# hbdat/cvpr22_cross_modal_pseudo_labeling

Measured on AMD Instinct MI355X. Metric: images/sec student-teacher train step (COCO 800x1333), higher is better.
Workload: dtype f32 (bf16x3 split MFMA, fp32 accum); 1 GPU; student_teacher_mask_rcnn_uncertainty.yaml R-50-C4, 2 img/GPU 3x800x1333, fwd+bwd+allreduce+SGD; global_batch=2, parallelism=dp1, losses_finite=True, pipelined=True

## Files before the change

### cvpr22_cross_modal_pseudo_labeling_amd/_C.py

```python
import contextlib
import functools
import ctypes
import threading

import torch

from . import _cpu, _lib

_L = _lib.load()


def _stream():
    return torch._C._cuda_getCurrentRawStream(torch.cuda.current_device())


class _Same:

    def __enter__(self):
        return None

    def __exit__(self, *exc):
        return False


# ... 789 lines not shown
        raise RuntimeError("split_gemm_pair: residual must be a float32 [M, N] HIP tensor with unit column stride")
    with _on(dev):
        config = _gemm_cfg(config)
        nbytes = _gemm_ws_bytes(m, n, ch, ch2, kh, kw, w, config) if not (config & 8) else 0
        ws = torch.empty((nbytes,), dtype=torch.uint8, device=dev) if nbytes else None
        rc = _L.ovis_split_gemm_pair(a_pair.data_ptr(), 2 * a_pair.stride(0),
                                     0 if a2_pair is None else a2_pair.data_ptr(),
                                     0 if a2_pair is None else 2 * a2_pair.stride(0),
                                     b_pair.data_ptr(), 2 * b_pair.stride(0),
                                     0 if c is None else c.data_ptr(), n, 0 if cp is None else cp.data_ptr(), 4 * n,
                                     0 if bias is None else bias.data_ptr(),
                                     0 if residual is None else residual.data_ptr(),
                                     0 if residual is None else residual.stride(0), m, n, ch, ch2, kh, kw, h, w,
                                     int(bool(flip)), int(bool(relu)), 0 if ws is None else ws.data_ptr(), nbytes,
                                     config, _stream())
    _lib.check(rc, "split_gemm_pair")
    return c, cp


def split_gemm_pair_pool_supported(m, n, ch, pool_rows):
    return bool(_L.ovis_split_gemm_pair_pool_supported(int(m), int(n), int(ch), int(pool_rows)))


def split_gemm_pair_rp_pool(a_pair, b_pair, bias, residual_pair, relu, out_f32, out_pair, pool_rows):
    for t, name in ((a_pair, "a_pair"), (b_pair, "b_pair")) + (((residual_pair, "residual_pair"),) if residual_pair is not None else ()):
        if not (t.is_cuda and t.dtype == torch.bfloat16 and t.dim() == 2 and t.stride(1) == 1):
            raise RuntimeError(f"split_gemm_pair_rp_pool: {name} must be a 2-D bfloat16 HIP tensor in pair layout")
    m, ch = a_pair.shape[0], a_pair.shape[1] // 2
    n, k = b_pair.shape[0], b_pair.shape[1] // 2
    if k != ch or m % pool_rows or (residual_pair is not None and residual_pair.shape != (m, 2 * n)):
        raise RuntimeError("split_gemm_pair_rp_pool: shape mismatch")
    dev = a_pair.device
    c = torch.empty((m, n), dtype=torch.float32, device=dev) if out_f32 else None
    cp = torch.empty((m, 2 * n), dtype=torch.bfloat16, device=dev) if out_pair else None
    pooled = torch.zeros((m // pool_rows, n), dtype=torch.float32, device=dev)
    if m == 0 or n == 0:
        return c, cp, pooled
    if bias is not None:
        bias = _dev(bias, "bias")
    with _on(dev):
        rc = _L.ovis_split_gemm_pair_rp_pool(a_pair.data_ptr(), 2 * a_pair.stride(0), b_pair.data_ptr(), 2 * b_pair.stride(0),
                                             0 if c is None else c.data_ptr(), n, 0 if cp is None else cp.data_ptr(), 4 * n,
                                             0 if bias is None else bias.data_ptr(),
                                             0 if residual_pair is None else residual_pair.data_ptr(),
                                             0 if residual_pair is None else 2 * residual_pair.stride(0), m, n, ch,
                                             int(bool(relu)), pooled.data_ptr(), int(pool_rows), 1.0 / pool_rows, _stream())
    _lib.check(rc, "split_gemm_pair_rp_pool")
    return c, cp, pooled


def weight_prep_pair(w, scale=None, want_transposed=False):
    if not (w.is_cuda and w.dtype == torch.float32 and w.dim() == 4):
        raise RuntimeError("weight_prep_pair: [N,C,KH,KW] float32 HIP tensor expected")
    w = w.detach().contiguous()
    n, c, kh, kw = w.shape
    t = kh * kw
    fwd = torch.empty((n, 2 * t * c), dtype=torch.bfloat16, device=w.device)
    bwd = torch.empty((c, 2 * t * n), dtype=torch.bfloat16, device=w.device) if want_transposed else None
    if scale is not None:
        scale = _dev(scale.detach(), "scale")
    with _on(w.device):
        rc = _L.ovis_weight_prep_pair_f32(w.data_ptr(), 0 if scale is None else scale.data_ptr(), fwd.data_ptr(),
                                          0 if bwd is None else bwd.data_ptr(), n, c, t, _stream())
    _lib.check(rc, "weight_prep_pair")
    return fwd, bwd


def split_gemm_pair_gated(a_pair, b_pair, gate_pair, conv=None, out_f32=False, out_pair=True, config=0):
    for t, name in ((a_pair, "a_pair"), (b_pair, "b_pair"), (gate_pair, "gate_pair")):
# ... 507 lines not shown
```

### cvpr22_cross_modal_pseudo_labeling_amd/_lib.py

```python
import ctypes
import os

_HERE = os.path.dirname(os.path.abspath(__file__))
LIB_PATH = os.path.join(_HERE, "libovis_hip.so")

OVIS_OK = 0
_ERRORS = {-1: "OVIS_EINVAL (bad size or null pointer)",
           -2: "OVIS_ENOSPC (workspace too small)",
           -3: "OVIS_ERANGE (problem size not supported by the kernel)"}

_vp, _i, _f, _sz, _l = ctypes.c_void_p, ctypes.c_int, ctypes.c_float, ctypes.c_size_t, ctypes.c_long

SIGNATURES = {
    "ovis_version": (ctypes.c_char_p, []),
    "ovis_roi_align_forward_f32": (_i, [_vp, _vp, _vp, _i, _i, _i, _i, _i, _i, _i, _f, _i, _vp]),
    "ovis_roi_align_forward_workspace_bytes": (_sz, [_i, _i, _i]),
    "ovis_roi_align_forward_mfma_supported": (_i, [_i, _i, _i, _i]),
    "ovis_roi_align_forward_ws_f32": (_i, [_vp, _vp, _vp, _i, _i, _i, _i, _i, _i, _i, _f, _i, _vp, _sz, _vp]),
    "ovis_roi_align_forward_strided_from_nhwc_f32": (_i, [_vp, _vp, _vp, _i, _i, _i, _i, _i, _i, _i, _i, _f, _i, _i, _vp]),
    "ovis_roi_align_backward_f32": (_i, [_vp, _vp, _vp, _i, _i, _i, _i, _i, _i, _i, _f, _i, _vp]),
    "ovis_roi_align_backward_workspace_bytes": (_sz, [_i, _i, _i, _i]),
    "ovis_roi_align_backward_plane_supported": (_i, [_i, _i, _i, _i]),
    "ovis_roi_align_backward_ws_f32": (_i, [_vp, _vp, _vp, _i, _i, _i, _i, _i, _i, _i, _f, _i, _vp, _sz, _vp]),
    "ovis_roi_align_backward_strided_ws_f32": (_i, [_vp, _vp, _vp, _i, _i, _i, _i, _i, _i, _i, _i, _f, _i, _vp, _sz, _vp]),
# ... 19 lines not shown
    "ovis_topk_sorted_f32": (_i, [_vp, _l, _i, _i, _i, _vp, _vp, _vp, _sz, _vp]),
    "ovis_rpn_decode_f32": (_i, [_vp, _l, _l, _l, _vp, _vp, _vp, _i, _i, _i, _i, _f, _f, _f, _f, _f, _f, _f, _vp, _vp, _vp]),
    "ovis_sigmoid_focal_loss_forward_f32": (_i, [_vp, _vp, _vp, _i, _i, _f, _f, _vp]),
    "ovis_sigmoid_focal_loss_backward_f32": (_i, [_vp, _vp, _vp, _vp, _i, _i, _f, _f, _vp]),
    "ovis_split_bf16x3_f32": (_i, [_vp, _l, _vp, _l, _i, _i, _vp]),
    "ovis_im2col_split_bf16x3_f32": (_i, [_vp, _vp, _l, _i, _i, _i, _i, _i, _i, _vp]),
    "ovis_bias_act_f32": (_i, [_vp, _vp, _vp, _l, _i, _i, _vp]),
    "ovis_split_pair_f32": (_i, [_vp, _l, _vp, _l, _i, _vp]),
    "ovis_gate_split_pair_rows_f32": (_i, [_vp, _l, _vp, _i, _vp, _vp, _l, _i, _vp, _i, _vp, _vp, _vp]),
    "ovis_gate_split_pair_f32": (_i, [_vp, _l, _vp, _i, _vp, _vp, _l, _i, _vp, _i, _vp]),
    "ovis_im2col_nchw_pair_f32": (_i, [_vp, _vp] + [_i] * 9 + [_vp]),
    "ovis_weight_prep_pair_f32": (_i, [_vp, _vp, _vp, _vp, _i, _i, _i, _vp]),
    "ovis_slab_reduce_f32": (_i, [_vp, _vp, _vp, _i, _i, _i, _i, _vp]),
    "ovis_im2col_pair": (_i, [_vp, _vp, _l, _i, _i, _i, _i, _i, _vp]),
    "ovis_split_gemm_tn_slices": (_i, [_l, _i, _i, _i]),
    "ovis_split_gemm_pair_tn": (_i, [_vp, _l, _vp, _l, _vp, _i, _l, _i, _i, _i, _i, _i, _i, _vp]),
    "ovis_split_gemm_pair_gated": (_i, [_vp, _l, _vp, _l, _vp, _l, _vp, _l, _vp, _l, _l] + [_i] * 8 + [_vp]),
    "ovis_split_gemm_pair_gated_ws": (_i, [_vp, _l, _vp, _l, _vp, _l, _vp, _l, _vp, _l, _l] + [_i] * 7 + [_vp, _sz, _i, _vp]),
    "ovis_split_gemm_pair_workspace_bytes": (_sz, [_l, _i, _i, _i, _i, _i, _i]),
    "ovis_split_gemm_pair_workspace_bytes_ex": (_sz, [_l, _i, _i, _i, _i, _i, _i, _i]),
    "ovis_split_gemm_pair_rp_gated": (_i, [_vp, _l, _vp, _l, _vp, _l, _vp, _l, _vp, _l, _vp, _l, _l, _i, _i, _i, _vp]),
    "ovis_split_gemm_pair_pool_supported": (_i, [_l, _i, _i, _i]),
    "ovis_split_gemm_pair_rp_pool": (_i, [_vp, _l, _vp, _l, _vp, _l, _vp, _l, _vp, _vp, _l, _l, _i, _i, _i, _vp, _i, _f, _vp]),
    "ovis_split_gemm_pair_rp": (_i, [_vp, _l, _vp, _l, _vp, _l, _vp, _l, _vp, _vp, _l, _l, _i, _i, _i, _vp, _sz, _i, _vp]),
    "ovis_split_gemm_pair": (_i, [_vp, _l, _vp, _l, _vp, _l, _vp, _l, _vp, _l, _vp, _vp, _l, _l] + [_i] * 9
                             + [_vp, _sz, _i, _vp]),
    "ovis_match_encode_f32": (_i, [_vp, _vp, _vp, _i, _i, _f, _f, _i, _f, _f, _f, _f, _vp, _vp, _vp, _vp]),
    "ovis_rpn_match_encode_f32": (_i, [_vp, _vp, _vp, _i, _i, _f, _f, _i, _f, _f, _f, _f, _vp, _vp, _vp, _vp]),
    "ovis_project_masks_f32": (_i, [_vp, _vp, _vp, _i, _i, _i, _i, _i, _vp, _vp]),
    "ovis_gemm_f32": (_i, [_vp, _l, _l, _vp, _l, _l, _vp, _vp, _l, _i, _i, _i, _vp]),
    "ovis_gemm_ex_f32": (_i, [_vp, _l, _l, _vp, _l, _l, _vp, _i, _f, _i, _vp, _l, _i, _i, _i, _vp]),
    "ovis_gemm_f32_workspace_bytes": (_sz, [_i, _i, _i]),
    "ovis_gemm_ex_ws_f32": (_i, [_vp, _l, _l, _vp, _l, _l, _vp, _i, _f, _i, _vp, _l, _i, _i, _i, _vp, _sz, _vp]),
    "ovis_deform_im2col_f32": (_i, [_vp, _vp, _vp, _vp] + [_i] * 13 + [_vp]),
    "ovis_deform_col2im_f32": (_i, [_vp, _vp, _vp, _vp] + [_i] * 13 + [_vp]),
    "ovis_deform_col2im_coord_f32": (_i, [_vp, _vp, _vp, _vp, _vp, _vp] + [_i] * 13 + [_vp]),
    "ovis_deform_im2col_pair_rows_f32": (_i, [_vp, _vp, _vp, _vp, _l] + [_i] * 15 + [_vp]),
    "ovis_deform_col2im_rows_f32": (_i, [_vp, _l, _vp, _vp, _vp, _vp, _vp, _vp] + [_i] * 15 + [_vp]),
    "ovis_region_noun_align_f32": (_i, [_vp, _vp, _vp, _vp, _vp, _i, _i, _i, _vp]),
    "ovis_text_embed_f32": (_i, [_vp, _l, _i, _vp, _vp, _i, _i, _vp, _vp]),
    "ovis_project_polygon_masks_f32": (_i, [_vp, _vp, _vp, _vp, _vp, _i, _i, _i, _i, _vp, _vp]),
    "ovis_sgd_momentum_multi_f32": (_i, [_vp, _vp, _i, _f, _f, _f, _i, _vp]),
    "ovis_bottleneck_identity_backward_workspace_bytes": (_sz, [_l, _i, _i, _i, _i, _i, _i]),
    "ovis_bottleneck_identity_backward": (_i, [_vp, _l] * 7 + [_vp] * 3 + [_l, _i, _i, _i, _i, _i, _i] + [_vp] * 7 + [_sz, _i, _vp, _vp]),
    "ovis_weight_prep_pair_multi_f32": (_i, [_vp, _vp, _i, _i, _vp]),
    "ovis_weight_prep_tile": (_i, []),
# ... 32 lines not shown
```

### cvpr22_cross_modal_pseudo_labeling_amd/csrc/split_gemm.hip

```cpp
#include <stdlib.h>

#include "ovis_common.h"
constexpr int kGroupWidth = 4;

namespace {
typedef short bf16x8 __attribute__((ext_vector_type(8)));
typedef float f32x4 __attribute__((ext_vector_type(4)));
typedef __bf16 b2 __attribute__((ext_vector_type(2)));
typedef float f2 __attribute__((ext_vector_type(2)));

__device__ char g_zero_line[128];

enum { PLAIN = 0, SHIFTED = 1, HALO = 2, DEFORM = 3 };
constexpr int kHalo = 8;

struct SplitGemmArgs {
  const char* A; long a_rs;
  const char* A2; long a2_rs;
  const char* B; long b_rs;
  float* C; long ldc;
  char* Cp; long cp_rs;
  const float* bias; const float* res; long ldr;
  const char* resp; long resp_rs;
  const char* gate; long gate_rs;
// ... 67 lines not shown
  }
  if (p.C) *(f32x4*)(p.C + m * p.ldc + n) = v;
  if (p.Cp) {
    const unsigned h01 = pack_bf16(v.x, v.y), h23 = pack_bf16(v.z, v.w);
    const unsigned l01 = pack_bf16(v.x - __uint_as_float(h01 << 16), v.y - __uint_as_float(h01 & 0xffff0000u));
    const unsigned l23 = pack_bf16(v.z - __uint_as_float(h23 << 16), v.w - __uint_as_float(h23 & 0xffff0000u));
    char* d = p.Cp + m * p.cp_rs + poff;
    *(uint2*)d = make_uint2(h01, h23);
    *(uint2*)(d + 64) = make_uint2(l01, l23);
  }
  return v;
}

__device__ __forceinline__ void epilogue_store4(const SplitGemmArgs& p, long m, int n, f32x4 v) {
  const long poff = (long)(n >> 5) * 128 + (n & 31) * 2;
  f32x4 bias4 = {0.f, 0.f, 0.f, 0.f};
  if (p.bias) bias4 = *(const f32x4*)(p.bias + n);
  const EpilogueSource src = epilogue_source(p);
  EpilogueOperands o;
  if (src.base) epilogue_fetch4(src, m, epilogue_column_bytes(p, n, poff), o);
  epilogue_apply4(p, m, n, poff, v, bias4, o);
}

template <int WM, int WN, int MODE, int NS, int OCC, bool DUAL = false, bool POOL = false>
__global__ __launch_bounds__(WM * WN * 64, OCC) void split_gemm_kernel(SplitGemmArgs p, int tiles_n, int ntiles) {
  constexpr int BM = WM * 64, BN = WN * 64, NW = WM * WN;
  constexpr int A_ROWS = MODE == HALO ? BM + 2 * kHalo + 2 : BM;
  constexpr int ZROW = BM + 2 * kHalo;
  constexpr int A_BYTES = A_ROWS * 128, B_BYTES = BN * 128, STAGE = A_BYTES + B_BYTES;
  constexpr int A_PIECES = (MODE == HALO ? BM + 2 * kHalo : BM) / 8;
  constexpr int AI = (A_PIECES + NW - 1) / NW;
  constexpr int BI = BN / 8 / NW;
  static_assert(MODE != HALO || NS == 1, "the halo tile is single-staged");
  static_assert(NW * 4096 <= STAGE * NS, "epilogue staging fits the k-loop's LDS");
  extern __shared__ __attribute__((aligned(16))) char smem[];

  const int lane = threadIdx.x & 63, wave = __builtin_amdgcn_readfirstlane(threadIdx.x >> 6);
  int id;
  {
    const int nblocks = gridDim.x;
    const int b = blockIdx.x, q = nblocks >> 3, r = nblocks & 7, xcd = b & 7, loc = b >> 3;
    id = (xcd < r ? xcd * (q + 1) : r * (q + 1) + (xcd - r) * q) + loc;
  }
  const int slice = id / ntiles;
  const int tile = id - slice * ntiles;
  const int gw = p.gw, tiles_m = ntiles / tiles_n;
  const int per_group = tiles_m * gw;
  const int grp = tile / per_group;
  const int in_grp = tile - grp * per_group;
  const int tile_m = in_grp / gw, tile_n = grp * gw + (in_grp - tile_m * gw);
  const long m0 = (long)tile_m * BM;
  const int n0 = tile_n * BN;
  const int Mi = (int)p.M;

  const int cpb = p.ch >> 5;
  const int nk = p.T * cpb + (p.ch2 >> 5);
  int dy = 0, dx = 0;
  auto set_tap = [&](int t) {
    dy = t / p.KW - p.KH / 2;
    dx = t % p.KW - p.KW / 2;
    if (p.flip) { dy = -dy; dx = -dx; }
  };

  struct LaneGeom { int lr, s0, s1; };
  auto lane_geom = [&](int ln) {
    const int lr = ln >> 3, lc = ln & 7;
// ... 328 lines not shown
              ps2 += rr >= pool_b2 ? fin : z;
            }
          }
        }
      }
    }
  }
  if constexpr (POOL) {
    f32x4* ps[3] = {&ps0, &ps1, &ps2};
#pragma unroll
    for (int sgm = 0; sgm < 3; ++sgm) {
      f32x4 v = *ps[sgm];
#pragma unroll
      for (int e = 0; e < 4; ++e) {
        v[e] += __shfl_xor(v[e], 16, 64);
        v[e] += __shfl_xor(v[e], 32, 64);
      }
      const long first = (m0 + wm * 64) + (sgm == 0 ? 0 : (sgm == 1 ? pool_b1 : pool_b2));
      if (er == 0 && col_ok && first < p.M && (sgm == 0 || (sgm == 1 ? pool_b1 : pool_b2) < 64)) {
        float* d = p.pool + (pool_map0 + sgm) * p.N + n;
#pragma unroll
        for (int e = 0; e < 4; ++e) atomicAdd(d + e, v[e] * p.pool_scale);
      }
    }
  }
}

__global__ __launch_bounds__(256) void split_gemm_finish_kernel(SplitGemmArgs p) {
  const int n4 = p.N >> 2;
  const long total = p.M * n4;
  const long slab = p.M * p.N;
  for (long i = (long)blockIdx.x * 256 + threadIdx.x; i < total; i += (long)gridDim.x * 256) {
    const long m = i / n4;
    const int n = (int)(i - m * n4) * 4;
    const float* s = p.slab + m * p.N + n;
    f32x4 v = *(const f32x4*)s;
    for (int k = 1; k < p.kslices; ++k) v += *(const f32x4*)(s + k * slab);
    epilogue_store4(p, m, n, v);
  }
}

typedef short bf16x4 __attribute__((ext_vector_type(4)));

struct SplitGemmTnArgs {
  const char* G; long g_rs;
  const char* X; long x_rs;
// ... 597 lines not shown
      attr_set_s = true;
    }
    hipLaunchKernelGGL((split_gemm_tn_kernel<true, true>), dim3((unsigned)nblocks), dim3(256), lds, s, p, tiles_i, tiles_j, (int)nblocks);
  } else if (T > 1) {
    static bool attr_set_c = false;
    if (!attr_set_c) {
      OVIS_HIP_TRY(hipFuncSetAttribute((const void*)split_gemm_tn_kernel<true>, hipFuncAttributeMaxDynamicSharedMemorySize, lds));
      attr_set_c = true;
    }
    hipLaunchKernelGGL(split_gemm_tn_kernel<true>, dim3((unsigned)nblocks), dim3(256), lds, s, p, tiles_i, tiles_j, (int)nblocks);
  } else {
    static bool attr_set = false;
    if (!attr_set) {
      OVIS_HIP_TRY(hipFuncSetAttribute((const void*)split_gemm_tn_kernel<false>, hipFuncAttributeMaxDynamicSharedMemorySize, lds));
      attr_set = true;
    }
    hipLaunchKernelGGL(split_gemm_tn_kernel<false>, dim3((unsigned)nblocks), dim3(256), lds, s, p, tiles_i, tiles_j, (int)nblocks);
  }
  OVIS_LAUNCH_CHECK();
  return OVIS_OK;
}

namespace {
struct SplitGemmPlan {
  int mode, narrow, stages, kslices, steps_per_slice, tiles_m, tiles_n;
};

SplitGemmPlan split_gemm_plan(long m, int n, int channels, int channels2, int taps_h, int taps_w, int width, int config) {
  SplitGemmPlan q;
  const int T = taps_h * taps_w;
  q.narrow = n <= 64;
  const int bn = q.narrow ? 64 : 128;
  q.tiles_m = (int)((m + 127) / 128);
  q.tiles_n = (n + bn - 1) / bn;
  const long nb = (long)q.tiles_m * q.tiles_n;
  q.mode = PLAIN;
  if (T > 1) q.mode = (!q.narrow && !(config & 4) && (taps_h / 2) * width + taps_w / 2 <= kHalo && T <= 16) ? HALO : SHIFTED;
  const int cpb = channels / 32;
  const int units = q.mode == HALO ? cpb : T * cpb + channels2 / 32;
  q.kslices = 1;
  q.steps_per_slice = units;
  bool sliced_two_stage = false;
  if (!(config & 8) && !q.narrow && nb <= OVIS_NUM_CU / 2) {
    const int min_units = q.mode == HALO ? 1 : 8;
    long s = units / min_units;
    const long want = (2L * OVIS_NUM_CU + nb - 1) / nb;
    if (s > want) s = want;
    if (s > 64) s = 64;
// ... 26 lines not shown
    if (best_sl > 1) {
      q.steps_per_slice = (units + best_sl - 1) / best_sl;
      q.kslices = (units + q.steps_per_slice - 1) / q.steps_per_slice;
      sliced_two_stage = true;
    }
  }
  if (const int forced = (config >> 8) & 0xff; forced > 0 && !q.narrow) {
    const int sl = forced < units ? forced : units;
    q.steps_per_slice = (units + sl - 1) / sl;
    q.kslices = (units + q.steps_per_slice - 1) / q.steps_per_slice;
  }
  const long total = nb * q.kslices;
  q.stages = 2;
  if (q.mode == HALO || q.narrow) q.stages = 1;
  else if (sliced_two_stage) q.stages = 2;
  else if (total >= 8L * OVIS_NUM_CU || (total >= 4L * OVIS_NUM_CU && (T > 1 || q.tiles_n >= 8))) q.stages = 1;
  else {
    const long slots2 = 2L * OVIS_NUM_CU, slots1 = 4L * OVIS_NUM_CU;
    if (total > slots2 && total <= slots2 + slots2 / 4 && total <= slots1) q.stages = 1;
    if (total > slots1 && total <= slots1 + slots1 / 16) q.stages = 1;
  }
  if (config & 1) q.stages = 1;
  if ((config & 2) && q.mode != HALO && !q.narrow) q.stages = 2;
  return q;
}
}

extern "C" size_t ovis_split_gemm_pair_workspace_bytes_ex(long m, int n, int channels, int channels2, int taps_h,
                                                          int taps_w, int width, int config) {
  if (m <= 0 || n <= 0 || channels <= 0 || taps_h <= 0 || taps_w <= 0 || config < 0 || config > 0x1ffff) return 0;
  const SplitGemmPlan q = split_gemm_plan(m, n, channels, channels2, taps_h, taps_w, width, config);
  return q.kslices > 1 ? (size_t)q.kslices * (size_t)m * (size_t)n * sizeof(float) : 0;
}

extern "C" size_t ovis_split_gemm_pair_workspace_bytes(long m, int n, int channels, int channels2, int taps_h,
                                                       int taps_w, int width) {
  return ovis_split_gemm_pair_workspace_bytes_ex(m, n, channels, channels2, taps_h, taps_w, width, 0);
}

static int split_gemm_pair_impl(const void* a_pair, long a_row_bytes, const void* a2_pair, long a2_row_bytes,
                                const void* b_pair, long b_row_bytes, float* c, long ldc, void* c_pair,
                                long c_pair_row_bytes, const float* bias, const float* residual, long ldr,
                                const void* residual_pair, long residual_pair_row_bytes,
                                const void* gate_pair, long gate_row_bytes, long m, int n, int channels, int channels2,
                                int taps_h, int taps_w, int height, int width, int flip, int relu, void* workspace,
                                size_t workspace_bytes, int config, void* stream, float* pool = nullptr, int pool_rows = 0,
// ... 18 lines not shown
  if (config < 0 || config > 0x1ffff) return OVIS_ERANGE;
  SplitGemmPlan q = split_gemm_plan(m, n, channels, channels2, taps_h, taps_w, width, config);
  if (q.kslices > 1 && (!workspace || workspace_bytes < (size_t)q.kslices * (size_t)m * (size_t)n * sizeof(float))) {
    q = split_gemm_plan(m, n, channels, channels2, taps_h, taps_w, width, config | 8);
  }
  SplitGemmArgs p;
  p.A = (const char*)a_pair; p.a_rs = a_row_bytes;
  p.A2 = (const char*)a2_pair; p.a2_rs = a2_row_bytes;
  p.B = (const char*)b_pair; p.b_rs = b_row_bytes;
  p.C = c; p.ldc = ldc; p.Cp = (char*)c_pair; p.cp_rs = c_pair_row_bytes;
  p.bias = bias; p.res = residual; p.ldr = ldr;
  p.resp = (const char*)residual_pair; p.resp_rs = residual_pair_row_bytes;
  p.gate = (const char*)gate_pair; p.gate_rs = gate_row_bytes;
  p.slab = q.kslices > 1 ? (float*)workspace : nullptr;
  p.pool = pool; p.pool_rows = pool_rows; p.pool_scale = pool_scale;
  p.M = m; p.N = n; p.ch = channels; p.ch2 = channels2; p.T = T; p.H = height; p.W = width; p.KH = taps_h; p.KW = taps_w;
  p.flip = flip; p.relu = relu;
  p.kslices = q.kslices; p.steps_per_slice = q.steps_per_slice;
  p.gw = (q.tiles_n % kGroupWidth == 0) ? kGroupWidth : (q.tiles_n % 4 == 0) ? 4 : q.tiles_n;
  const long ntiles = (long)q.tiles_m * q.tiles_n;
  const long nblocks = ntiles * q.kslices;
  if (nblocks > 0x7fffffffL) return OVIS_ERANGE;
  hipStream_t s = (hipStream_t)stream;
#define OVIS_SG_LAUNCH__(WM_, WN_, MODE_, NS_, OCC_, DUAL_, POOL_)                                                   \
  do {                                                                                                              \
    constexpr int a_rows = MODE_ == HALO ? WM_ * 64 + 2 * kHalo + 2 : WM_ * 64;                                      \
    constexpr int lds = NS_ * (a_rows * 128 + WN_ * 64 * 128);                                                       \
    static bool attr_set = false;                                                                                   \
    if (!attr_set) {                                                                                                \
      OVIS_HIP_TRY(hipFuncSetAttribute((const void*)split_gemm_kernel<WM_, WN_, MODE_, NS_, OCC_, DUAL_, POOL_>,    \
                                       hipFuncAttributeMaxDynamicSharedMemorySize, lds));                           \
      attr_set = true;                                                                                              \
    }                                                                                                               \
    hipLaunchKernelGGL((split_gemm_kernel<WM_, WN_, MODE_, NS_, OCC_, DUAL_, POOL_>), dim3((unsigned)nblocks),      \
                       dim3(WM_ * WN_ * 64), lds, s, p, q.tiles_n, (int)ntiles);                                    \
  } while (0)
#define OVIS_SG_LAUNCH_(WM_, WN_, MODE_, NS_, OCC_, DUAL_) OVIS_SG_LAUNCH__(WM_, WN_, MODE_, NS_, OCC_, DUAL_, false)
#define OVIS_SG_LAUNCH(WM_, WN_, MODE_, NS_, OCC_) OVIS_SG_LAUNCH_(WM_, WN_, MODE_, NS_, OCC_, false)
  if (pool) {
    if (dual || q.narrow || q.mode != PLAIN || q.kslices > 1) return OVIS_ERANGE;
    if (q.stages == 1) OVIS_SG_LAUNCH__(2, 2, PLAIN, 1, 4, false, true); else OVIS_SG_LAUNCH__(2, 2, PLAIN, 2, 2, false, true);
  } else if (dual) {
    if (q.narrow || q.mode != PLAIN || q.kslices > 1) return OVIS_ERANGE;
    if (q.stages == 1) OVIS_SG_LAUNCH_(2, 2, PLAIN, 1, 4, true); else OVIS_SG_LAUNCH_(2, 2, PLAIN, 2, 2, true);
  } else if (q.narrow) {
    if (q.mode == PLAIN) OVIS_SG_LAUNCH(2, 1, PLAIN, 1, 2); else OVIS_SG_LAUNCH(2, 1, SHIFTED, 1, 2);
  } else if (q.mode == HALO) {
    OVIS_SG_LAUNCH(2, 2, HALO, 1, 4);
  } else if (q.mode == SHIFTED) {
    if (q.stages == 1) OVIS_SG_LAUNCH(2, 2, SHIFTED, 1, 4); else OVIS_SG_LAUNCH(2, 2, SHIFTED, 2, 2);
  } else {
    if (q.stages == 1) OVIS_SG_LAUNCH(2, 2, PLAIN, 1, 4); else OVIS_SG_LAUNCH(2, 2, PLAIN, 2, 2);
  }
#undef OVIS_SG_LAUNCH__
#undef OVIS_SG_LAUNCH_
#undef OVIS_SG_LAUNCH
  OVIS_LAUNCH_CHECK();
  if (q.kslices > 1) {
    p.slab = (float*)workspace;
    const long total = m * (n / 4);
    const long blocks = (total + 255) / 256;
    const unsigned grid = (unsigned)(blocks < 8L * OVIS_NUM_CU ? blocks : 8L * OVIS_NUM_CU);
    hipLaunchKernelGGL(split_gemm_finish_kernel, dim3(grid), dim3(256), 0, s, p);
    OVIS_LAUNCH_CHECK();
  }
  return OVIS_OK;
}

extern "C" int ovis_split_gemm_pair(const void* a_pair, long a_row_bytes, const void* a2_pair, long a2_row_bytes,
                                    const void* b_pair, long b_row_bytes, float* c, long ldc, void* c_pair,
                                    long c_pair_row_bytes, const float* bias, const float* residual, long ldr, long m,
                                    int n, int channels, int channels2, int taps_h, int taps_w, int height, int width,
                                    int flip, int relu, void* workspace, size_t workspace_bytes, int config,
                                    void* stream) {
  return split_gemm_pair_impl(a_pair, a_row_bytes, a2_pair, a2_row_bytes, b_pair, b_row_bytes, c, ldc, c_pair,
                              c_pair_row_bytes, bias, residual, ldr, nullptr, 0, nullptr, 0, m, n, channels, channels2,
                              taps_h, taps_w, height, width, flip, relu, workspace, workspace_bytes, config, stream);
}

extern "C" int ovis_split_gemm_pair_rp(const void* a_pair, long a_row_bytes, const void* b_pair, long b_row_bytes,
                                       float* c, long ldc, void* c_pair, long c_pair_row_bytes, const float* bias,
                                       const void* residual_pair, long residual_pair_row_bytes, long m, int n,
                                       int channels, int relu, void* workspace, size_t workspace_bytes, int config,
                                       void* stream) {
  if (!residual_pair || n % 32 != 0 || residual_pair_row_bytes % 16 != 0 || ((uintptr_t)residual_pair & 15)) return OVIS_ERANGE;
  return split_gemm_pair_impl(a_pair, a_row_bytes, nullptr, 0, b_pair, b_row_bytes, c, ldc, c_pair, c_pair_row_bytes, bias,
                              nullptr, 0, residual_pair, residual_pair_row_bytes, nullptr, 0, m, n, channels, 0, 1, 1, 0, 0,
                              0, relu, workspace, workspace_bytes, config, stream);
}

extern "C" int ovis_split_gemm_pair_pool_supported(long m, int n, int channels, int pool_rows) {
  if (m <= 0 || n <= 0 || channels <= 0 || channels % 32 || n % 32 || pool_rows < 32 || pool_rows > 64) return 0;
  const SplitGemmPlan q = split_gemm_plan(m, n, channels, 0, 1, 1, 0, 0);
  return !q.narrow && q.mode == PLAIN && q.kslices == 1;
}

extern "C" int ovis_split_gemm_pair_rp_pool(const void* a_pair, long a_row_bytes, const void* b_pair, long b_row_bytes,
                                            float* c, long ldc, void* c_pair, long c_pair_row_bytes, const float* bias,
                                            const void* residual_pair, long residual_pair_row_bytes, long m, int n,
                                            int channels, int relu, float* pooled, int pool_rows, float pool_scale,
                                            void* stream) {
  if (!pooled) return OVIS_EINVAL;
  if (n % 32 != 0 || (residual_pair && (residual_pair_row_bytes % 16 != 0 || ((uintptr_t)residual_pair & 15)))) return OVIS_ERANGE;
  return split_gemm_pair_impl(a_pair, a_row_bytes, nullptr, 0, b_pair, b_row_bytes, c, ldc, c_pair, c_pair_row_bytes, bias,
                              nullptr, 0, residual_pair, residual_pair_row_bytes, nullptr, 0, m, n, channels, 0, 1, 1, 0, 0,
                              0, relu, nullptr, 0, 8, stream, pooled, pool_rows, pool_scale);
}

extern "C" int ovis_split_gemm_pair_gated(const void* a_pair, long a_row_bytes, const void* b_pair, long b_row_bytes,
                                          float* c, long ldc, void* c_pair, long c_pair_row_bytes,
                                          const void* gate_pair, long gate_row_bytes, long m, int n, int channels,
                                          int taps_h, int taps_w, int height, int width, int flip, int config,
                                          void* stream) {
  if (!gate_pair || gate_row_bytes % 16 != 0 || ((uintptr_t)gate_pair & 15) || n % 32 != 0) return OVIS_ERANGE;
  return split_gemm_pair_impl(a_pair, a_row_bytes, nullptr, 0, b_pair, b_row_bytes, c, ldc, c_pair, c_pair_row_bytes,
                              nullptr, nullptr, 0, nullptr, 0, gate_pair, gate_row_bytes, m, n, channels, 0, taps_h, taps_w,
                              height, width, flip, 0, nullptr, 0, config | 8, stream);
}

extern "C" int ovis_split_gemm_pair_gated_ws(const void* a_pair, long a_row_bytes, const void* b_pair, long b_row_bytes,
                                             float* c, long ldc, void* c_pair, long c_pair_row_bytes,
                                             const void* gate_pair, long gate_row_bytes, long m, int n, int channels,
                                             int taps_h, int taps_w, int height, int width, int flip, void* workspace,
                                             size_t workspace_bytes, int config, void* stream) {
  if (!gate_pair || gate_row_bytes % 16 != 0 || ((uintptr_t)gate_pair & 15) || n % 32 != 0) return OVIS_ERANGE;
  return split_gemm_pair_impl(a_pair, a_row_bytes, nullptr, 0, b_pair, b_row_bytes, c, ldc, c_pair, c_pair_row_bytes,
                              nullptr, nullptr, 0, nullptr, 0, gate_pair, gate_row_bytes, m, n, channels, 0, taps_h, taps_w,
                              height, width, flip, 0, workspace, workspace_bytes, config, stream);
}
// ... 58 lines not shown
```

### include/ovis_hip.h

```cpp
#ifndef OVIS_HIP_H_
#define OVIS_HIP_H_

#include <stddef.h>
#include <stdint.h>

#ifdef __cplusplus
extern "C" {
#endif

#define OVIS_OK 0
#define OVIS_EINVAL (-1)
#define OVIS_ENOSPC (-2)
#define OVIS_ERANGE (-3)

const char* ovis_version(void);

int ovis_roi_align_forward_f32(const float* input, const float* rois, float* output,
                               int num_rois, int batch, int channels, int height,
                               int width, int pooled_h, int pooled_w,
                               float spatial_scale, int sampling_ratio, void* stream);

size_t ovis_roi_align_forward_workspace_bytes(int num_rois, int height, int width);
int ovis_roi_align_forward_mfma_supported(int height, int width, int pooled_h, int pooled_w);
int ovis_roi_align_forward_ws_f32(const float* input, const float* rois, float* output,
// ... 127 lines not shown
int ovis_split_gemm_pair_gated(const void* a_pair, long a_row_bytes, const void* b_pair, long b_row_bytes,
                               float* c, long ldc, void* c_pair, long c_pair_row_bytes, const void* gate_pair,
                               long gate_row_bytes, long m, int n, int channels, int taps_h, int taps_w,
                               int height, int width, int flip, int config, void* stream);

int ovis_split_gemm_pair_gated_ws(const void* a_pair, long a_row_bytes, const void* b_pair, long b_row_bytes,
                                  float* c, long ldc, void* c_pair, long c_pair_row_bytes, const void* gate_pair,
                                  long gate_row_bytes, long m, int n, int channels, int taps_h, int taps_w,
                                  int height, int width, int flip, void* workspace, size_t workspace_bytes,
                                  int config, void* stream);

int ovis_split_gemm_pair_rp_gated(const void* a_pair, long a_row_bytes, const void* b_pair, long b_row_bytes, float* c,
                                  long ldc, void* c_pair, long c_pair_row_bytes, const void* residual_pair,
                                  long residual_pair_row_bytes, const void* gate_pair, long gate_row_bytes, long m, int n,
                                  int channels, int config, void* stream);

int ovis_im2col_nchw_pair_f32(const float* src, void* dst_pair, int num, int channels, int height, int width,
                              int kh, int kw, int stride, int pad, int k_padded, void* stream);

size_t ovis_split_gemm_pair_workspace_bytes(long m, int n, int channels, int channels2, int taps_h, int taps_w,
                                            int width);
size_t ovis_split_gemm_pair_workspace_bytes_ex(long m, int n, int channels, int channels2, int taps_h, int taps_w,
                                               int width, int config);
int ovis_split_gemm_pair(const void* a_pair, long a_row_bytes, const void* a2_pair, long a2_row_bytes,
                         const void* b_pair, long b_row_bytes, float* c, long ldc, void* c_pair,
                         long c_pair_row_bytes, const float* bias, const float* residual, long ldr, long m,
                         int n, int channels, int channels2, int taps_h, int taps_w, int height, int width,
                         int flip, int relu, void* workspace, size_t workspace_bytes, int config, void* stream);
int ovis_split_gemm_pair_rp(const void* a_pair, long a_row_bytes, const void* b_pair, long b_row_bytes, float* c, long ldc,
                            void* c_pair, long c_pair_row_bytes, const float* bias, const void* residual_pair,
                            long residual_pair_row_bytes, long m, int n, int channels, int relu, void* workspace,
                            size_t workspace_bytes, int config, void* stream);

int ovis_split_gemm_tn_slices(long m, int n, int channels, int taps);
int ovis_split_gemm_pair_tn(const void* g_pair, long g_row_bytes, const void* x_pair, long x_row_bytes,
                            float* c_slabs, int slices, long m, int n, int channels, int taps_h,
                            int taps_w, int height, int width, void* stream);

int ovis_match_encode_f32(const float* gt_boxes, const int64_t* gt_labels, const float* proposals, int num_gt,
                          int num_proposals, float high_threshold, float low_threshold, int between_keeps_label,
                          float wx, float wy, float ww, float wh, int64_t* matched_idx, int64_t* labels,
                          float* regression_targets, void* stream);
int ovis_rpn_match_encode_f32(const float* gt_boxes, const float* anchors, const uint8_t* visibility, int num_gt,
                              int num_anchors, float high_threshold, float low_threshold, int allow_low_quality_matches,
                              float wx, float wy, float ww, float wh, uint32_t* best_per_gt_scratch, int64_t* labels,
                              float* regression_targets, void* stream);
// ... 64 lines not shown

int ovis_text_embed_f32(const float* table, long table_rows, int dim, const int32_t* input_ids,
                        const int32_t* special_tokens_mask, int num_words, int max_tokens, float* out, void* stream);

int ovis_project_polygon_masks_f32(const float* coords, const int32_t* polygon_start, const int32_t* instance_start,
                                   const int64_t* gt_index, const float* boxes, int num, int image_width,
                                   int image_height, int resolution, float* out, void* stream);

int ovis_deform_im2col_pair_rows_f32(const float* input_nhwc, const float* offset, const float* mask, void* columns_pair,
                                     long columns_row_bytes, int batch, int channels, int height, int width, int out_h,
                                     int out_w, int kernel_h, int kernel_w, int stride_h, int stride_w, int pad_h, int pad_w,
                                     int dil_h, int dil_w, int deformable_group, void* stream);
int ovis_deform_col2im_rows_f32(const float* dcol_rows, long dcol_ld, const float* input_nhwc, const float* offset,
                                const float* mask, float* grad_input_nhwc, float* grad_offset, float* grad_mask, int batch,
                                int channels, int height, int width, int out_h, int out_w, int kernel_h, int kernel_w,
                                int stride_h, int stride_w, int pad_h, int pad_w, int dil_h, int dil_w, int deformable_group,
                                void* stream);

int ovis_split_gemm_pair_pool_supported(long m, int n, int channels, int pool_rows);
int ovis_split_gemm_pair_rp_pool(const void* a_pair, long a_row_bytes, const void* b_pair, long b_row_bytes, float* c,
                                 long ldc, void* c_pair, long c_pair_row_bytes, const float* bias,
                                 const void* residual_pair, long residual_pair_row_bytes, long m, int n, int channels,
                                 int relu, float* pooled, int pool_rows, float pool_scale, void* stream);

int ovis_sgd_momentum_multi_f32(const void* items, const void* blocks, int num_blocks, float lr, float weight_decay,
                                float momentum, int apply_weight_decay, void* stream);
int ovis_sgd_chunk_elements(void);

size_t ovis_bottleneck_identity_backward_workspace_bytes(long m, int channels, int mid_channels, int taps_h, int taps_w,
                                                         int width, int config);
int ovis_bottleneck_identity_backward(
    const void* g3_pair, long g3_row_bytes, const void* x_pair, long x_row_bytes, const void* o1_pair, long o1_row_bytes,
    const void* o2_pair, long o2_row_bytes, const void* t1_pair, long t1_row_bytes, const void* t2_pair, long t2_row_bytes,
    const void* t3_pair, long t3_row_bytes, const float* scale1, const float* scale2, const float* scale3, long m, int channels,
    int mid_channels, int taps_h, int taps_w, int height, int width, void* g2_pair, void* g1_pair, void* gx_pair, float* dw1,
    float* dw2, float* dw3, void* workspace, size_t workspace_bytes, int config, void* stream, void* side_stream);

int ovis_weight_prep_pair_multi_f32(const void* items, const void* blocks, int num_blocks, int max_taps, void* stream);
int ovis_weight_prep_tile(void);

#ifdef __cplusplus
}
#endif
#endif
```

Baseline: 60.71 images/sec.

## Add persistent tile-loop variant of split GEMM for large plain single-stage products

Splits the split-GEMM kernel body into a per-tile device function and adds a persistent launch mode. In that mode a grid of OCC×CU blocks loops over tiles, keeping each XCD's contiguous tile range. The mode is chosen automatically for plain, non-narrow, single-stage, unsliced products with many blocks and short k-loops. The aim is to cut block launch and scheduling overhead on GEMMs with many small tiles. The cost is an extra barrier per tile and possible load imbalance. The pooled path only uses persistence when it is explicitly requested through a config bit.

```diff
diff --git a/cvpr22_cross_modal_pseudo_labeling_amd/_C.py b/cvpr22_cross_modal_pseudo_labeling_amd/_C.py
--- a/cvpr22_cross_modal_pseudo_labeling_amd/_C.py
+++ b/cvpr22_cross_modal_pseudo_labeling_amd/_C.py
@@ -835,7 +835,12 @@
     return bool(_L.ovis_split_gemm_pair_pool_supported(int(m), int(n), int(ch), int(pool_rows)))
 
 
-def split_gemm_pair_rp_pool(a_pair, b_pair, bias, residual_pair, relu, out_f32, out_pair, pool_rows):
+def split_gemm_pair_persistent_chosen(m, n, ch, ch2=0, conv=None, config=0):
+    w, kh, kw = (conv[1], conv[2], conv[3]) if conv is not None else (0, 1, 1)
+    return bool(_L.ovis_split_gemm_pair_persistent_chosen(int(m), int(n), int(ch), int(ch2), kh, kw, w, int(config)))
+
+
+def split_gemm_pair_rp_pool(a_pair, b_pair, bias, residual_pair, relu, out_f32, out_pair, pool_rows, config=0):
     for t, name in ((a_pair, "a_pair"), (b_pair, "b_pair")) + (((residual_pair, "residual_pair"),) if residual_pair is not None else ()):
         if not (t.is_cuda and t.dtype == torch.bfloat16 and t.dim() == 2 and t.stride(1) == 1):
             raise RuntimeError(f"split_gemm_pair_rp_pool: {name} must be a 2-D bfloat16 HIP tensor in pair layout")
@@ -852,12 +857,14 @@
     if bias is not None:
         bias = _dev(bias, "bias")
     with _on(dev):
-        rc = _L.ovis_split_gemm_pair_rp_pool(a_pair.data_ptr(), 2 * a_pair.stride(0), b_pair.data_ptr(), 2 * b_pair.stride(0),
-                                             0 if c is None else c.data_ptr(), n, 0 if cp is None else cp.data_ptr(), 4 * n,
-                                             0 if bias is None else bias.data_ptr(),
-                                             0 if residual_pair is None else residual_pair.data_ptr(),
-                                             0 if residual_pair is None else 2 * residual_pair.stride(0), m, n, ch,
-                                             int(bool(relu)), pooled.data_ptr(), int(pool_rows), 1.0 / pool_rows, _stream())
+        rc = _L.ovis_split_gemm_pair_rp_pool_cfg(a_pair.data_ptr(), 2 * a_pair.stride(0), b_pair.data_ptr(),
+                                                 2 * b_pair.stride(0), 0 if c is None else c.data_ptr(), n,
+                                                 0 if cp is None else cp.data_ptr(), 4 * n,
+                                                 0 if bias is None else bias.data_ptr(),
+                                                 0 if residual_pair is None else residual_pair.data_ptr(),
+                                                 0 if residual_pair is None else 2 * residual_pair.stride(0), m, n, ch,
+                                                 int(bool(relu)), pooled.data_ptr(), int(pool_rows), 1.0 / pool_rows,
+                                                 _gemm_cfg(config), _stream())
     _lib.check(rc, "split_gemm_pair_rp_pool")
     return c, cp, pooled
 
diff --git a/cvpr22_cross_modal_pseudo_labeling_amd/_lib.py b/cvpr22_cross_modal_pseudo_labeling_amd/_lib.py
--- a/cvpr22_cross_modal_pseudo_labeling_amd/_lib.py
+++ b/cvpr22_cross_modal_pseudo_labeling_amd/_lib.py
@@ -65,6 +65,8 @@
     "ovis_split_gemm_pair_rp_gated": (_i, [_vp, _l, _vp, _l, _vp, _l, _vp, _l, _vp, _l, _vp, _l, _l, _i, _i, _i, _vp]),
     "ovis_split_gemm_pair_pool_supported": (_i, [_l, _i, _i, _i]),
     "ovis_split_gemm_pair_rp_pool": (_i, [_vp, _l, _vp, _l, _vp, _l, _vp, _l, _vp, _vp, _l, _l, _i, _i, _i, _vp, _i, _f, _vp]),
+    "ovis_split_gemm_pair_rp_pool_cfg": (_i, [_vp, _l, _vp, _l, _vp, _l, _vp, _l, _vp, _vp, _l, _l, _i, _i, _i, _vp, _i, _f, _i, _vp]),
+    "ovis_split_gemm_pair_persistent_chosen": (_i, [_l, _i, _i, _i, _i, _i, _i, _i]),
     "ovis_split_gemm_pair_rp": (_i, [_vp, _l, _vp, _l, _vp, _l, _vp, _l, _vp, _vp, _l, _l, _i, _i, _i, _vp, _sz, _i, _vp]),
     "ovis_split_gemm_pair": (_i, [_vp, _l, _vp, _l, _vp, _l, _vp, _l, _vp, _l, _vp, _vp, _l, _l] + [_i] * 9
                              + [_vp, _sz, _i, _vp]),
diff --git a/cvpr22_cross_modal_pseudo_labeling_amd/csrc/split_gemm.hip b/cvpr22_cross_modal_pseudo_labeling_amd/csrc/split_gemm.hip
--- a/cvpr22_cross_modal_pseudo_labeling_amd/csrc/split_gemm.hip
+++ b/cvpr22_cross_modal_pseudo_labeling_amd/csrc/split_gemm.hip
@@ -113,8 +113,8 @@
   epilogue_apply4(p, m, n, poff, v, bias4, o);
 }
 
-template <int WM, int WN, int MODE, int NS, int OCC, bool DUAL = false, bool POOL = false>
-__global__ __launch_bounds__(WM * WN * 64, OCC) void split_gemm_kernel(SplitGemmArgs p, int tiles_n, int ntiles) {
+template <int WM, int WN, int MODE, int NS, int OCC, bool DUAL, bool POOL, bool PERSIST>
+__device__ __forceinline__ void split_gemm_tile(const SplitGemmArgs& p, int tiles_n, int ntiles, int id) {
   constexpr int BM = WM * 64, BN = WN * 64, NW = WM * WN;
   constexpr int A_ROWS = MODE == HALO ? BM + 2 * kHalo + 2 : BM;
   constexpr int ZROW = BM + 2 * kHalo;
@@ -124,15 +124,12 @@
   constexpr int BI = BN / 8 / NW;
   static_assert(MODE != HALO || NS == 1, "the halo tile is single-staged");
   static_assert(NW * 4096 <= STAGE * NS, "epilogue staging fits the k-loop's LDS");
+  static_assert(!PERSIST || (MODE == PLAIN && NS == 1), "the tile loop exists for plain single-stage products");
   extern __shared__ __attribute__((aligned(16))) char smem[];
 
-  const int lane = threadIdx.x & 63, wave = __builtin_amdgcn_readfirstlane(threadIdx.x >> 6);
-  int id;
-  {
-    const int nblocks = gridDim.x;
-    const int b = blockIdx.x, q = nblocks >> 3, r = nblocks & 7, xcd = b & 7, loc = b >> 3;
-    id = (xcd < r ? xcd * (q + 1) : r * (q + 1) + (xcd - r) * q) + loc;
-  }
+  int lane_id = threadIdx.x & 63;
+  if constexpr (PERSIST) asm volatile("" : "+v"(lane_id));
+  const int lane = lane_id, wave = __builtin_amdgcn_readfirstlane(threadIdx.x >> 6);
   const int slice = id / ntiles;
   const int tile = id - slice * ntiles;
   const int gw = p.gw, tiles_m = ntiles / tiles_n;
@@ -507,6 +504,25 @@
 #pragma unroll
         for (int e = 0; e < 4; ++e) atomicAdd(d + e, v[e] * p.pool_scale);
       }
+    }
+  }
+}
+
+template <int WM, int WN, int MODE, int NS, int OCC, bool DUAL = false, bool POOL = false, bool PERSIST = false>
+__global__ __launch_bounds__(WM * WN * 64, OCC) void split_gemm_kernel(SplitGemmArgs p, int tiles_n, int ntiles) {
+  const int nblocks = gridDim.x;
+  const int b = blockIdx.x, q = nblocks >> 3, r = nblocks & 7, xcd = b & 7, loc = b >> 3;
+  if constexpr (!PERSIST) {
+    const int id = (xcd < r ? xcd * (q + 1) : r * (q + 1) + (xcd - r) * q) + loc;
+    split_gemm_tile<WM, WN, MODE, NS, OCC, DUAL, POOL, false>(p, tiles_n, ntiles, id);
+  } else {
+    const int tq = ntiles >> 3, tr = ntiles & 7;
+    const int first = xcd < tr ? xcd * (tq + 1) : tr * (tq + 1) + (xcd - tr) * tq;
+    const int end = first + tq + (xcd < tr ? 1 : 0);
+    const int step = q + (xcd < r ? 1 : 0);
+    for (int t = first + loc; t < end; t += step) {
+      split_gemm_tile<WM, WN, MODE, NS, OCC, DUAL, POOL, true>(p, tiles_n, ntiles, t);
+      __syncthreads();
     }
   }
 }
@@ -1150,8 +1166,10 @@
 }
 
 namespace {
+constexpr int kPersistMaxSteps = 32;
 struct SplitGemmPlan {
   int mode, narrow, stages, kslices, steps_per_slice, tiles_m, tiles_n;
+  int persist;
 };
 
 SplitGemmPlan split_gemm_plan(long m, int n, int channels, int channels2, int taps_h, int taps_w, int width, int config) {
@@ -1224,6 +1242,11 @@
   }
   if (config & 1) q.stages = 1;
   if ((config & 2) && q.mode != HALO && !q.narrow) q.stages = 2;
+  q.persist = 0;
+  if (q.mode == PLAIN && !q.narrow && q.stages == 1 && q.kslices == 1 && !(config & 0x20)) {
+    const bool chosen = nb >= 8L * OVIS_NUM_CU && units <= kPersistMaxSteps && !(config & 0x10000);
+    q.persist = chosen || (config & 0x10);
+  }
   return q;
 }
 }
@@ -1288,27 +1311,33 @@
   const long nblocks = ntiles * q.kslices;
   if (nblocks > 0x7fffffffL) return OVIS_ERANGE;
   hipStream_t s = (hipStream_t)stream;
-#define OVIS_SG_LAUNCH__(WM_, WN_, MODE_, NS_, OCC_, DUAL_, POOL_)                                                   \
+#define OVIS_SG_LAUNCH___(WM_, WN_, MODE_, NS_, OCC_, DUAL_, POOL_, PERSIST_)                                         \
   do {                                                                                                              \
     constexpr int a_rows = MODE_ == HALO ? WM_ * 64 + 2 * kHalo + 2 : WM_ * 64;                                      \
     constexpr int lds = NS_ * (a_rows * 128 + WN_ * 64 * 128);                                                       \
     static bool attr_set = false;                                                                                   \
     if (!attr_set) {                                                                                                \
-      OVIS_HIP_TRY(hipFuncSetAttribute((const void*)split_gemm_kernel<WM_, WN_, MODE_, NS_, OCC_, DUAL_, POOL_>,    \
-                                       hipFuncAttributeMaxDynamicSharedMemorySize, lds));                           \
+      OVIS_HIP_TRY(hipFuncSetAttribute(                                                                             \
+          (const void*)split_gemm_kernel<WM_, WN_, MODE_, NS_, OCC_, DUAL_, POOL_, PERSIST_>,                       \
+          hipFuncAttributeMaxDynamicSharedMemorySize, lds));                                                        \
       attr_set = true;                                                                                              \
     }                                                                                                               \
-    hipLaunchKernelGGL((split_gemm_kernel<WM_, WN_, MODE_, NS_, OCC_, DUAL_, POOL_>), dim3((unsigned)nblocks),      \
+    const long grid = PERSIST_ ? (long)OCC_ * OVIS_NUM_CU : nblocks;    \
+    hipLaunchKernelGGL((split_gemm_kernel<WM_, WN_, MODE_, NS_, OCC_, DUAL_, POOL_, PERSIST_>), dim3((unsigned)grid), \
                        dim3(WM_ * WN_ * 64), lds, s, p, q.tiles_n, (int)ntiles);                                    \
   } while (0)
+#define OVIS_SG_LAUNCH__(WM_, WN_, MODE_, NS_, OCC_, DUAL_, POOL_) OVIS_SG_LAUNCH___(WM_, WN_, MODE_, NS_, OCC_, DUAL_, POOL_, false)
 #define OVIS_SG_LAUNCH_(WM_, WN_, MODE_, NS_, OCC_, DUAL_) OVIS_SG_LAUNCH__(WM_, WN_, MODE_, NS_, OCC_, DUAL_, false)
 #define OVIS_SG_LAUNCH(WM_, WN_, MODE_, NS_, OCC_) OVIS_SG_LAUNCH_(WM_, WN_, MODE_, NS_, OCC_, false)
   if (pool) {
+    if (!(config & 0x10)) q.persist = 0;
     if (dual || q.narrow || q.mode != PLAIN || q.kslices > 1) return OVIS_ERANGE;
-    if (q.stages == 1) OVIS_SG_LAUNCH__(2, 2, PLAIN, 1, 4, false, true); else OVIS_SG_LAUNCH__(2, 2, PLAIN, 2, 2, false, true);
+    if (q.persist) OVIS_SG_LAUNCH___(2, 2, PLAIN, 1, 3, false, true, true);
+    else if (q.stages == 1) OVIS_SG_LAUNCH__(2, 2, PLAIN, 1, 4, false, true); else OVIS_SG_LAUNCH__(2, 2, PLAIN, 2, 2, false, true);
   } else if (dual) {
     if (q.narrow || q.mode != PLAIN || q.kslices > 1) return OVIS_ERANGE;
-    if (q.stages == 1) OVIS_SG_LAUNCH_(2, 2, PLAIN, 1, 4, true); else OVIS_SG_LAUNCH_(2, 2, PLAIN, 2, 2, true);
+    if (q.persist) OVIS_SG_LAUNCH___(2, 2, PLAIN, 1, 4, true, false, true);
+    else if (q.stages == 1) OVIS_SG_LAUNCH_(2, 2, PLAIN, 1, 4, true); else OVIS_SG_LAUNCH_(2, 2, PLAIN, 2, 2, true);
   } else if (q.narrow) {
     if (q.mode == PLAIN) OVIS_SG_LAUNCH(2, 1, PLAIN, 1, 2); else OVIS_SG_LAUNCH(2, 1, SHIFTED, 1, 2);
   } else if (q.mode == HALO) {
@@ -1316,8 +1345,10 @@
   } else if (q.mode == SHIFTED) {
     if (q.stages == 1) OVIS_SG_LAUNCH(2, 2, SHIFTED, 1, 4); else OVIS_SG_LAUNCH(2, 2, SHIFTED, 2, 2);
   } else {
-    if (q.stages == 1) OVIS_SG_LAUNCH(2, 2, PLAIN, 1, 4); else OVIS_SG_LAUNCH(2, 2, PLAIN, 2, 2);
-  }
+    if (q.persist) OVIS_SG_LAUNCH___(2, 2, PLAIN, 1, 4, false, false, true);
+    else if (q.stages == 1) OVIS_SG_LAUNCH(2, 2, PLAIN, 1, 4); else OVIS_SG_LAUNCH(2, 2, PLAIN, 2, 2);
+  }
+#undef OVIS_SG_LAUNCH___
 #undef OVIS_SG_LAUNCH__
 #undef OVIS_SG_LAUNCH_
 #undef OVIS_SG_LAUNCH
@@ -1361,16 +1392,33 @@
   return !q.narrow && q.mode == PLAIN && q.kslices == 1;
 }
 
+extern "C" int ovis_split_gemm_pair_rp_pool_cfg(const void* a_pair, long a_row_bytes, const void* b_pair, long b_row_bytes,
+                                                float* c, long ldc, void* c_pair, long c_pair_row_bytes, const float* bias,
+                                                const void* residual_pair, long residual_pair_row_bytes, long m, int n,
+                                                int channels, int relu, float* pooled, int pool_rows, float pool_scale,
+                                                int config, void* stream) {
+  if (!pooled) return OVIS_EINVAL;
+  if (n % 32 != 0 || (residual_pair && (residual_pair_row_bytes % 16 != 0 || ((uintptr_t)residual_pair & 15)))) return OVIS_ERANGE;
+  if (config < 0 || config > 0x1ffff) return OVIS_ERANGE;
+  return split_gemm_pair_impl(a_pair, a_row_bytes, nullptr, 0, b_pair, b_row_bytes, c, ldc, c_pair, c_pair_row_bytes, bias,
+                              nullptr, 0, residual_pair, residual_pair_row_bytes, nullptr, 0, m, n, channels, 0, 1, 1, 0, 0,
+                              0, relu, nullptr, 0, config | 8, stream, pooled, pool_rows, pool_scale);
+}
+
 extern "C" int ovis_split_gemm_pair_rp_pool(const void* a_pair, long a_row_bytes, const void* b_pair, long b_row_bytes,
                                             float* c, long ldc, void* c_pair, long c_pair_row_bytes, const float* bias,
                                             const void* residual_pair, long residual_pair_row_bytes, long m, int n,
                                             int channels, int relu, float* pooled, int pool_rows, float pool_scale,
                                             void* stream) {
-  if (!pooled) return OVIS_EINVAL;
-  if (n % 32 != 0 || (residual_pair && (residual_pair_row_bytes % 16 != 0 || ((uintptr_t)residual_pair & 15)))) return OVIS_ERANGE;
-  return split_gemm_pair_impl(a_pair, a_row_bytes, nullptr, 0, b_pair, b_row_bytes, c, ldc, c_pair, c_pair_row_bytes, bias,
-                              nullptr, 0, residual_pair, residual_pair_row_bytes, nullptr, 0, m, n, channels, 0, 1, 1, 0, 0,
-                              0, relu, nullptr, 0, 8, stream, pooled, pool_rows, pool_scale);
+  return ovis_split_gemm_pair_rp_pool_cfg(a_pair, a_row_bytes, b_pair, b_row_bytes, c, ldc, c_pair, c_pair_row_bytes, bias,
+                                          residual_pair, residual_pair_row_bytes, m, n, channels, relu, pooled, pool_rows,
+                                          pool_scale, 0, stream);
+}
+
+extern "C" int ovis_split_gemm_pair_persistent_chosen(long m, int n, int channels, int channels2, int taps_h, int taps_w,
+                                                      int width, int config) {
+  if (m <= 0 || n <= 0 || channels <= 0 || taps_h <= 0 || taps_w <= 0 || config < 0 || config > 0x1ffff) return 0;
+  return split_gemm_plan(m, n, channels, channels2, taps_h, taps_w, width, config).persist != 0;
 }
 
 extern "C" int ovis_split_gemm_pair_gated(const void* a_pair, long a_row_bytes, const void* b_pair, long b_row_bytes,
diff --git a/include/ovis_hip.h b/include/ovis_hip.h
--- a/include/ovis_hip.h
+++ b/include/ovis_hip.h
@@ -173,6 +173,8 @@
                                             int width);
 size_t ovis_split_gemm_pair_workspace_bytes_ex(long m, int n, int channels, int channels2, int taps_h, int taps_w,
                                                int width, int config);
+int ovis_split_gemm_pair_persistent_chosen(long m, int n, int channels, int channels2, int taps_h, int taps_w, int width,
+                                           int config);
 int ovis_split_gemm_pair(const void* a_pair, long a_row_bytes, const void* a2_pair, long a2_row_bytes,
                          const void* b_pair, long b_row_bytes, float* c, long ldc, void* c_pair,
                          long c_pair_row_bytes, const float* bias, const float* residual, long ldr, long m,
@@ -283,6 +285,10 @@
                                  long ldc, void* c_pair, long c_pair_row_bytes, const float* bias,
                                  const void* residual_pair, long residual_pair_row_bytes, long m, int n, int channels,
                                  int relu, float* pooled, int pool_rows, float pool_scale, void* stream);
+int ovis_split_gemm_pair_rp_pool_cfg(const void* a_pair, long a_row_bytes, const void* b_pair, long b_row_bytes, float* c,
+                                     long ldc, void* c_pair, long c_pair_row_bytes, const float* bias,
+                                     const void* residual_pair, long residual_pair_row_bytes, long m, int n, int channels,
+                                     int relu, float* pooled, int pool_rows, float pool_scale, int config, void* stream);
 
 int ovis_sgd_momentum_multi_f32(const void* items, const void* blocks, int num_blocks, float lr, float weight_decay,
                                 float momentum, int apply_weight_decay, void* stream);
```

Result: slower. 59.81 images/sec (-1.5%).
